# intel/neural-compressor

Hardware: AMD Instinct MI355X
Metric: llama2_7b_gptq_int4_g128_quantize_wall_clock (lower is better)
Workload: dtype bf16

## Files before the change

### include/inc_mi355x.h

```cpp
#ifndef INC_MI355X_H_
#define INC_MI355X_H_

#include <stdint.h>

#ifdef __cplusplus
extern "C" {
#endif

#define INC_OK 0
#define INC_ERR_BAD_ARG (-1)
#define INC_ERR_UNSUPPORTED (-2)
#define INC_ERR_LAUNCH (-3)
#define INC_ERR_WORKSPACE (-4)

#define INC_F32 0
#define INC_F16 1
#define INC_BF16 2

#define INC_SCHEME_ASYM 0
#define INC_SCHEME_SYM 1

typedef void* inc_stream_t;

int inc_abi_version(void);
// ... 122 lines not shown
int inc_gptq_hessian_accum_routed(const void* a, int xdtype, int mode, const int32_t* route, int64_t T, int top_k, int64_t E,
                                  int64_t K, float* H, int64_t* rows, inc_stream_t stream);

int inc_gptq_hessian_finalize(float* H, int64_t K, float percdamp, uint8_t* dead, void* workspace,
                              inc_stream_t stream);

int inc_gptq_prepare_weight(const void* w, int wdtype, float* out, const uint8_t* dead, int64_t N,
                            int64_t K, inc_stream_t stream);

int inc_gptq_find_params(const float* w, int64_t N, int64_t K, int64_t col0, int group_size,
                         int ngroups, int bits, int sym, float* scale, float* zero, int64_t G,
                         int64_t g0, inc_stream_t stream);

int inc_gptq_find_params_mse(const float* w, int64_t N, int64_t K, int64_t col0, int group_size,
                             int ngroups, int bits, int sym, int grid, float maxshrink, float norm,
                             float* scale, float* zero, int64_t G, int64_t g0, inc_stream_t stream);

int inc_gptq_quant_block(const float* w, const float* Hinv, const float* scale, const float* zero,
                         uint8_t* codes, void* q_out, int q_dtype, float* err, int64_t N, int64_t K,
                         int64_t G, int64_t i1, int count, int group_size, int bits,
                         inc_stream_t stream);

int inc_gptq_quant_block_params(const float* w, const float* Hinv, float* scale, float* zero,
                                uint8_t* codes, void* q_out, int q_dtype, float* err, int64_t N, int64_t K,
                                int64_t G, int64_t i1, int count, int group_size, int bits, int sym,
                                inc_stream_t stream);

int inc_gptq_lazy_update(float* w, const float* Hinv, const float* err, int64_t N, int64_t K,
                         int64_t i1, int count, inc_stream_t stream);

int inc_gptq_lazy_update_cols(float* w, const float* Hinv, const float* err, int64_t N, int64_t K,
                              int64_t i1, int count, int64_t col_begin, int64_t col_end,
                              inc_stream_t stream);

#define INC_GPTQ_DYNAMIC_GROUPS 1
#define INC_GPTQ_MSE 2
#define INC_GPTQ_NO_LOOKAHEAD 4
#define INC_GPTQ_NO_FUSED_PARAMS 8
int inc_gptq_quantize_layer(float* w, const float* Hinv, float* scale, float* zero, int64_t G,
                            const float* loop_scale, const float* loop_zero, int64_t loop_G, uint8_t* codes,
                            void* q_out, int q_dtype, float* err_ws, int64_t N, int64_t K, int group_size,
                            int kernel_group_size, int block_size, int bits, int sym, int flags,
                            inc_stream_t stream, inc_stream_t aux_stream);

int inc_chol_diag_block(float* A, int64_t lda, int n, float* Linv, int64_t ldi, int32_t* info, int tag,
                        inc_stream_t stream);

int64_t inc_gptq_inverse_factor_workspace_bytes(int64_t K, int flags);
int inc_gptq_inverse_factor(const float* H, int64_t K, float* U, void* workspace, int64_t workspace_bytes, int32_t* info,
                            int flags, inc_stream_t stream, inc_stream_t aux_stream);

int inc_awq_act_abs_sum(const void* x, int xdtype, int64_t T, int64_t K, float* out,
                        inc_stream_t stream);
int64_t inc_awq_weight_scale_workspace_bytes(int64_t N, int64_t K, int group_size);
int inc_awq_weight_scale(const void* w, int wdtype, int64_t N, int64_t K, int group_size, float* out,
                         void* workspace, int64_t workspace_bytes, inc_stream_t stream);

int inc_awq_repack(const int32_t* awq_qweight, const int32_t* awq_qzeros, int64_t K, int64_t N, int64_t G, int bits,
                   int32_t* qweight, int32_t* qzeros, inc_stream_t stream);

int64_t inc_w8a8_gemm_workspace_bytes(int64_t M, int64_t N, int64_t K);
int inc_sq_channel_minmax(const void* x, int xdtype, int64_t T, int64_t K, int64_t ld, float* mn, float* mx,
                          inc_stream_t stream);
int inc_sq_weight_col_absmax(const void* w, int wdtype, int64_t N, int64_t K, float* out, inc_stream_t stream);
int inc_sq_cal_scale(const float* amax_x, const float* amax_w, int64_t K, float alpha, float weight_max_lb, float* scale,
                     inc_stream_t stream);
int inc_sq_quant_weight(const void* w, int wdtype, int64_t N, int64_t K, int64_t Kp, const float* smooth, int8_t* qw,
                        float* w_scale, int32_t* rowsum, inc_stream_t stream);
int inc_sq_quant_act(const void* x, int xdtype, int64_t M, int64_t K, int64_t Kp, const float* in_scale, float sx, float zp,
                     int8_t* out, inc_stream_t stream);
int inc_w8a8_gemm(const int8_t* xq, const int8_t* wq, const float* alpha, const int32_t* corr, const void* bias, void* y,
                  int ydtype, int64_t M, int64_t N, int64_t K, void* workspace, int64_t workspace_bytes,
                  inc_stream_t stream);

int inc_probe_hbm_triad(float* a, const float* b, const float* c, float s, int64_t n, inc_stream_t stream);
int inc_probe_hbm_copy(void* dst, const void* src, int64_t bytes, int variant, inc_stream_t stream);
int inc_probe_mfma_bf16(const void* src, float* sink, int blocks, int iters, double* flops_out, inc_stream_t stream);
int inc_trace_marker(int id, inc_stream_t stream);

int inc_fwd_silu_mul(const void* gate, const void* up, void* out, int64_t n, int dtype, inc_stream_t stream);
int inc_fwd_rope(const void* q, const void* k, const void* cos, const void* sin, void* q_out, void* k_out, int64_t B, int64_t Hq,
                 int64_t Hk, int64_t T, int64_t D, const int64_t* strides, int64_t cs_batch, int dtype, inc_stream_t stream);
int inc_fwd_rmsnorm(const void* x, const void* w, void* out, int64_t rows, int64_t cols, float eps, int dtype, inc_stream_t stream);

#ifdef __cplusplus
}
#endif
#endif
```

### neural_compressor_amd/_lib.py

```python

import ctypes
import os
from ctypes import c_char_p, c_float, c_int, c_int64, c_void_p

_HERE = os.path.dirname(os.path.abspath(__file__))
LIB_PATH = os.path.join(_HERE, "libinc_mi355x.so")
ABI_VERSION = 12

INC_OK = 0
INC_F32, INC_F16, INC_BF16 = 0, 1, 2
INC_SCHEME_ASYM, INC_SCHEME_SYM = 0, 1

_P = c_void_p
SIGNATURES = {
    "inc_abi_version": (c_int, []),
    "inc_error_string": (c_char_p, [c_int]),
    "inc_target_arch": (c_char_p, []),
    "inc_pack_rows": (c_int, [_P, _P, c_int64, c_int64, c_int, c_int, _P]),
    "inc_unpack_rows": (c_int, [_P, _P, c_int64, c_int64, c_int, c_int, c_int, _P]),
    "inc_woq_pack": (c_int, [_P, c_int, _P, _P, _P, _P, _P, c_int64, c_int64, c_int64, c_int, c_int, _P]),
    "inc_woq_unpack": (c_int, [_P, _P, _P, _P, c_int64, c_int64, c_int64, c_int, _P, _P, _P]),
    "inc_woq_dequant": (c_int, [_P, _P, _P, _P, _P, c_int, c_int64, c_int64, c_int64, c_int, c_int, _P]),
    "inc_dequant_ints": (c_int, [_P, _P, c_int, _P, _P, _P, c_int, c_int64, c_int64, c_int64, c_int, _P]),
    "inc_woq_gemm_workspace_bytes": (c_int64, [c_int64, c_int64, c_int64]),
    "inc_woq_gemm": (
        c_int,
        [_P, c_int, _P, _P, _P, _P, _P, _P, c_int64, c_int64, c_int64, c_int64, c_int, c_int, _P, c_int64, _P],
    ),
    "inc_woq_gemm_route": (
        c_int,
        [c_int64, c_int64, c_int64, c_int, c_int, c_int, c_int, _P, _P, _P, _P, c_int64, _P, _P, _P, _P, _P, _P],
    ),
    "inc_woq_gemm_perm": (
        c_int,
        [_P, c_int, _P, _P, _P, _P, _P, _P, c_int64, c_int64, c_int64, c_int64, c_int, c_int, _P, c_int64, _P],
    ),
    "inc_woq_gemm_lut_workspace_bytes": (c_int64, [c_int64, c_int64, c_int64]),
    "inc_woq_gemm_lut": (
        c_int,
        [_P, c_int, _P, c_int64, _P, _P, c_int, c_int, _P, c_int64, _P, _P, c_int64, c_int64, c_int64, c_int64, c_int, _P, c_int64, _P],
    ),
    "inc_moe_route_bytes": (c_int64, [c_int64, c_int, c_int64]),
    "inc_moe_route": (c_int, [_P, c_int, c_int64, c_int, c_int64, _P, c_int64, _P]),
    "inc_woq_moe_gemm_workspace_bytes": (c_int64, [c_int, c_int64, c_int, c_int64, c_int64, c_int64]),
    "inc_woq_moe_gemm": (
        c_int,
        [c_int, _P, c_int, _P, _P, _P, _P, _P, c_int, _P, c_int64, c_int, c_int64, c_int64, c_int64, c_int64, c_int, _P, c_int64, _P],
    ),
    "inc_moe_combine": (c_int, [_P, _P, _P, c_int, c_int64, c_int, c_int64, c_int64, _P]),
    "inc_woq_gemm_multi_workspace_bytes": (c_int64, [c_int, c_int64, _P, c_int64]),
    "inc_woq_gemm_multi": (c_int, [c_int, _P, c_int, _P, _P, _P, _P, _P, c_int64, _P, c_int64, c_int, c_int, _P, c_int64, _P]),
    "inc_woq_gemm_multi_perm": (c_int, [c_int, _P, c_int, _P, _P, _P, _P, _P, _P, c_int64, _P, c_int64, c_int, c_int, _P, c_int64, _P]),
    "inc_woq_gemm_gated_workspace_bytes": (c_int64, [c_int64, c_int64, c_int64]),
    "inc_woq_gemm_gated": (
        c_int,
        [_P, c_int, _P, _P, _P, _P, _P, _P, _P, _P, _P, c_int64, c_int64, c_int64, c_int, c_int, c_int, _P, c_int64, _P],
    ),
    "inc_woq_gemv_anyw_slices": (c_int, [c_int64, c_int64, c_int64, c_int]),
    "inc_woq_gemv_anyw_workspace_bytes": (c_int64, [c_int64, c_int64, c_int64, c_int]),
    "inc_woq_gemv_anyw": (c_int, [_P, c_int, _P, _P, _P, _P, _P, c_int64, c_int64, c_int64, c_int64, c_int, c_int, _P, c_int64, _P]),
    "inc_woq_gemv_anyw_perm": (c_int, [_P, c_int, _P, _P, _P, _P, _P, _P, c_int64, c_int64, c_int64, c_int64, c_int, c_int, _P, c_int64, _P]),
    "inc_woq_gemv_anyw_multi_workspace_bytes": (c_int64, [c_int, c_int64, _P, c_int64, c_int]),
    "inc_woq_gemv_anyw_multi": (c_int, [c_int, _P, c_int, _P, _P, _P, _P, _P, _P, c_int64, _P, c_int64, c_int, c_int, _P, c_int64, _P]),
    "inc_groupwise_quant": (
        c_int,
        [_P, c_int, _P, _P, _P, _P, c_int64, c_int64, c_int, c_int, c_int, c_float, c_int, _P],
    ),
    "inc_codebook_quant": (c_int, [_P, c_int, _P, _P, _P, c_int64, c_int64, c_int, _P, _P, c_int, c_float, _P]),
    "inc_codebook_quant_with_scale": (c_int, [_P, c_int, _P, _P, _P, c_int64, c_int64, c_int, _P, _P, c_int, c_float, _P, _P]),
    "inc_mse_accumulate_workspace_bytes": (c_int64, []),
    "inc_mse_accumulate": (c_int, [_P, _P, c_int, c_int64, _P, _P, _P]),
    "inc_gptq_hessian_accum": (c_int, [_P, c_int, c_int64, c_int64, c_int64, _P, c_float, c_float, _P]),
    "inc_gptq_hessian_accum_multi": (c_int, [c_int, _P, c_int, c_int64, _P, _P, _P, _P, _P, _P, c_int64, _P]),
    "inc_gptq_hessian_accum_multi_workspace_bytes": (c_int64, []),
    "inc_gptq_hessian_accum_routed": (c_int, [_P, c_int, c_int, _P, c_int64, c_int, c_int64, c_int64, _P, _P, _P]),
    "inc_gptq_hessian_finalize": (c_int, [_P, c_int64, c_float, _P, _P, _P]),
    "inc_gptq_prepare_weight": (c_int, [_P, c_int, _P, _P, c_int64, c_int64, _P]),
    "inc_gptq_find_params": (
        c_int,
        [_P, c_int64, c_int64, c_int64, c_int, c_int, c_int, c_int, _P, _P, c_int64, c_int64, _P],
    ),
    "inc_sq_channel_minmax": (c_int, [_P, c_int, c_int64, c_int64, c_int64, _P, _P, _P]),
    "inc_sq_weight_col_absmax": (c_int, [_P, c_int, c_int64, c_int64, _P, _P]),
    "inc_sq_cal_scale": (c_int, [_P, _P, c_int64, c_float, c_float, _P, _P]),
    "inc_sq_quant_weight": (c_int, [_P, c_int, c_int64, c_int64, c_int64, _P, _P, _P, _P, _P]),
    "inc_sq_quant_act": (c_int, [_P, c_int, c_int64, c_int64, c_int64, _P, c_float, c_float, _P, _P]),
    "inc_w8a8_gemm_workspace_bytes": (c_int64, [c_int64, c_int64, c_int64]),
    "inc_w8a8_gemm": (c_int, [_P, _P, _P, _P, _P, _P, c_int, c_int64, c_int64, c_int64, _P, c_int64, _P]),
    "inc_awq_repack": (c_int, [_P, _P, c_int64, c_int64, c_int64, c_int, _P, _P, _P]),
    "inc_gptq_find_params_mse": (
        c_int,
        [_P, c_int64, c_int64, c_int64, c_int, c_int, c_int, c_int, c_int, c_float, c_float, _P, _P, c_int64, c_int64, _P],
    ),
    "inc_gptq_quant_block": (
        c_int,
        [_P, _P, _P, _P, _P, _P, c_int, _P, c_int64, c_int64, c_int64, c_int64, c_int, c_int, c_int, _P],
    ),
    "inc_gptq_quant_block_params": (c_int, [_P, _P, _P, _P, _P, _P, c_int, _P, c_int64, c_int64, c_int64, c_int64, c_int, c_int, c_int, c_int, _P]),
    "inc_gptq_lazy_update": (c_int, [_P, _P, _P, c_int64, c_int64, c_int64, c_int, _P]),
    "inc_gptq_lazy_update_cols": (c_int, [_P, _P, _P, c_int64, c_int64, c_int64, c_int, c_int64, c_int64, _P]),
    "inc_probe_hbm_triad": (c_int, [_P, _P, _P, c_float, c_int64, _P]),
    "inc_probe_hbm_copy": (c_int, [_P, _P, c_int64, c_int, _P]),
    "inc_probe_mfma_bf16": (c_int, [_P, _P, c_int, c_int, _P, _P]),
    "inc_trace_marker": (c_int, [c_int, _P]),
    "inc_gptq_quantize_layer": (c_int, [_P, _P, _P, _P, c_int64, _P, _P, c_int64, _P, _P, c_int, _P, c_int64, c_int64, c_int, c_int, c_int,
                                        c_int, c_int, c_int, _P, _P]),
    "inc_chol_diag_block": (c_int, [_P, c_int64, c_int, _P, c_int64, _P, c_int, _P]),
    "inc_gptq_inverse_factor_workspace_bytes": (c_int64, [c_int64, c_int]),
    "inc_gptq_inverse_factor": (c_int, [_P, c_int64, _P, _P, c_int64, _P, c_int, _P, _P]),
    "inc_awq_act_abs_sum": (c_int, [_P, c_int, c_int64, c_int64, _P, _P]),
    "inc_awq_weight_scale_workspace_bytes": (c_int64, [c_int64, c_int64, c_int]),
    "inc_awq_weight_scale": (c_int, [_P, c_int, c_int64, c_int64, c_int, _P, _P, c_int64, _P]),
    "inc_fwd_silu_mul": (c_int, [_P, _P, _P, c_int64, c_int, _P]),
    "inc_fwd_rope": (c_int, [_P, _P, _P, _P, _P, _P, c_int64, c_int64, c_int64, c_int64, c_int64, _P, c_int64, c_int, _P]),
    "inc_fwd_rmsnorm": (c_int, [_P, _P, _P, c_int64, c_int64, c_float, c_int, _P]),
}


class IncLibraryError(RuntimeError):
    """Raised when libinc_mi355x.so is missing, stale, or a call returns an INC_ERR_* code."""


def _load():
    if not os.path.exists(LIB_PATH):
        raise IncLibraryError(
            f"{LIB_PATH} not found. The MI355X HIP extension is mandatory (there is no CPU fallback): "
            "build it with `python -c 'import __graft_entry__ as g; g.build()'` or "
            "`make -C neural_compressor_amd/csrc`."
        )
    lib = ctypes.CDLL(LIB_PATH)
    for name, (restype, argtypes) in SIGNATURES.items():
        try:
            fn = getattr(lib, name)
        except AttributeError as e:
            raise IncLibraryError(f"{LIB_PATH} does not export `{name}`; rebuild the extension") from e
        fn.restype = restype
        fn.argtypes = argtypes
    got = lib.inc_abi_version()
    if got != ABI_VERSION:
        raise IncLibraryError(f"ABI mismatch: library reports {got}, bindings expect {ABI_VERSION}; rebuild")
    return lib


lib = _load()


def check(code, what):
    if code != INC_OK:
        msg = lib.inc_error_string(code).decode()
        raise IncLibraryError(f"{what} failed: {msg} (code {code})")
```

### neural_compressor_amd/csrc/fwd_elementwise.hip

```cpp
#include "common.hpp"

namespace {

typedef uint32_t u32x4 __attribute__((ext_vector_type(4)));

template <int DT>
__device__ __forceinline__ uint16_t t_round(float f) {
  if constexpr (DT == INC_BF16) {
    uint32_t u = __float_as_uint(f);
    if ((u & 0x7fffffffu) > 0x7f800000u) return 0x7FC0;
    u += 0x7fffu + ((u >> 16) & 1u);
    return static_cast<uint16_t>(u >> 16);
  } else {
    return f32_to_f16_bits(f);
  }
}
template <int DT>
__device__ __forceinline__ float t_f32(uint16_t b) {
  if constexpr (DT == INC_BF16) return bf16_bits_to_f32(b);
  else return f16_bits_to_f32(b);
}
template <int DT>
__device__ __forceinline__ float t_rf(float f) { return t_f32<DT>(t_round<DT>(f)); }

template <int DT>
__device__ __forceinline__ void unpack8(const u32x4 v, float (&e)[8]) {
#pragma unroll
  for (int i = 0; i < 4; ++i) {
    e[2 * i] = t_f32<DT>(static_cast<uint16_t>(v[i] & 0xffffu));
    e[2 * i + 1] = t_f32<DT>(static_cast<uint16_t>(v[i] >> 16));
  }
}
__device__ __forceinline__ u32x4 pack8(const uint16_t (&b)[8]) {
  u32x4 v;
#pragma unroll
  for (int i = 0; i < 4; ++i) v[i] = static_cast<uint32_t>(b[2 * i]) | (static_cast<uint32_t>(b[2 * i + 1]) << 16);
  return v;
}
__device__ __forceinline__ u32x4 ld_nt(const void* p, int64_t i16) { return __builtin_nontemporal_load(static_cast<const u32x4*>(p) + i16); }
__device__ __forceinline__ void st_nt(void* p, int64_t i16, u32x4 v) { __builtin_nontemporal_store(v, static_cast<u32x4*>(p) + i16); }

template <int DT>
__device__ __forceinline__ uint16_t silu_mul_one(float g, float u) {
#pragma clang fp contract(off)
  const float s = t_rf<DT>(g / (1.0f + expf(-g)));
  return t_round<DT>(s * u);
}

template <int DT>
__global__ __launch_bounds__(256) void fwd_silu_mul_kernel(const void* __restrict__ gate, const void* __restrict__ up, void* __restrict__ out, int64_t n) {
  const int64_t n8 = n >> 3;
  const int64_t i = (int64_t)blockIdx.x * 256 + threadIdx.x;
  if (i < n8) {
    float g[8], u[8];
    unpack8<DT>(ld_nt(gate, i), g);
    unpack8<DT>(ld_nt(up, i), u);
    uint16_t r[8];
#pragma unroll
    for (int e = 0; e < 8; ++e) r[e] = silu_mul_one<DT>(g[e], u[e]);
    st_nt(out, i, pack8(r));
  } else {
    const int64_t e = n8 * 8 + (i - n8);
    if (e < n) {
      const uint16_t* g = static_cast<const uint16_t*>(gate);
      const uint16_t* u = static_cast<const uint16_t*>(up);
      static_cast<uint16_t*>(out)[e] = silu_mul_one<DT>(t_f32<DT>(g[e]), t_f32<DT>(u[e]));
    }
  }
}

struct RopeStrides {
  int64_t q[3], k[3], qo[3], ko[3];
};

template <int DT>
__global__ __launch_bounds__(256) void fwd_rope_kernel(const void* __restrict__ q, const void* __restrict__ k, const void* __restrict__ cosp,
                                                       const void* __restrict__ sinp, void* __restrict__ q_out, void* __restrict__ k_out,
                                                       uint32_t total, uint32_t Hq, uint32_t Hk, uint32_t T, uint32_t D, uint32_t cs_batch,
                                                       RopeStrides st) {
#pragma clang fp contract(off)
  const uint32_t idx = blockIdx.x * 256u + threadIdx.x;
  if (idx >= total) return;
  const uint32_t d16 = D >> 4, H = Hq + Hk;
  const uint32_t dc = idx % d16;
  uint32_t r = idx / d16;
  const uint32_t hh = r % H;
  r /= H;
  const uint32_t t = r % T, b = r / T;
  const bool is_k = hh >= Hq;
  const uint32_t h = is_k ? hh - Hq : hh;
  const int64_t* si = is_k ? st.k : st.q;
  const int64_t* so = is_k ? st.ko : st.qo;
  const char* src = static_cast<const char*>(is_k ? k : q);
  char* dst = static_cast<char*>(is_k ? k_out : q_out);
  const int64_t in_off = (int64_t)b * si[0] + (int64_t)h * si[1] + (int64_t)t * si[2] + dc * 8;
  const int64_t out_off = (int64_t)b * so[0] + (int64_t)h * so[1] + (int64_t)t * so[2] + dc * 8;
  const int64_t cs_off = ((int64_t)(cs_batch == 1 ? 0 : b) * T + t) * D + dc * 8;
  const int64_t half = D >> 1;

  float lo[8], hi[8], c_lo[8], c_hi[8], s_lo[8], s_hi[8];
  unpack8<DT>(ld_nt(src, in_off >> 3), lo);
  unpack8<DT>(ld_nt(src, (in_off + half) >> 3), hi);
  unpack8<DT>(static_cast<const u32x4*>(cosp)[cs_off >> 3], c_lo);
  unpack8<DT>(static_cast<const u32x4*>(cosp)[(cs_off + half) >> 3], c_hi);
  unpack8<DT>(static_cast<const u32x4*>(sinp)[cs_off >> 3], s_lo);
  unpack8<DT>(static_cast<const u32x4*>(sinp)[(cs_off + half) >> 3], s_hi);
  uint16_t o_lo[8], o_hi[8];
#pragma unroll
  for (int e = 0; e < 8; ++e) {
    o_lo[e] = t_round<DT>(t_rf<DT>(lo[e] * c_lo[e]) + t_rf<DT>(-hi[e] * s_lo[e]));
    o_hi[e] = t_round<DT>(t_rf<DT>(hi[e] * c_hi[e]) + t_rf<DT>(lo[e] * s_hi[e]));
  }
  st_nt(dst, out_off >> 3, pack8(o_lo));
  st_nt(dst, (out_off + half) >> 3, pack8(o_hi));
}

template <int DT, int WAVES, int J>
__global__ __launch_bounds__(WAVES == 1 ? 256 : 512) void fwd_rmsnorm_kernel(const void* __restrict__ x, const void* __restrict__ w, void* __restrict__ out,
                                                                              int64_t rows, int cols, float eps, float factor) {
#pragma clang fp contract(off)
  constexpr int HALVES = (WAVES == 1 ? 256 : 512) / 32, ROWS_PER_BLOCK = HALVES / WAVES;
  __shared__ float part[ROWS_PER_BLOCK][8];
  const int p = threadIdx.x & 31, hw = threadIdx.x >> 5;
  const int rb = hw / WAVES, tw = hw % WAVES;
  const int64_t row = (int64_t)blockIdx.x * ROWS_PER_BLOCK + rb;
  const bool live = row < rows;
  const int pieces = cols >> 3;
  const int64_t base = (live ? row : 0) * (int64_t)pieces;
  const int first = p + 32 * tw;

  u32x4 v[J];
#pragma unroll
  for (int j = 0; j < J; ++j) {
    const int u = first + 32 * WAVES * j;
    if (live && u < pieces) v[j] = ld_nt(x, base + u);
  }
  float a[4] = {0.f, 0.f, 0.f, 0.f}, b[4] = {0.f, 0.f, 0.f, 0.f};
#pragma unroll
  for (int j = 0; j < J; ++j) {
    const int u = first + 32 * WAVES * j;
    if (live && u < pieces) {
      float e[8];
      unpack8<DT>(v[j], e);
#pragma unroll
      for (int i = 0; i < 4; ++i) {
        a[i] = a[i] + e[i] * e[i];
        b[i] = b[i] + e[4 + i] * e[4 + i];
      }
    }
  }
  float s = (((a[0] + a[1]) + a[2]) + a[3]) + (((b[0] + b[1]) + b[2]) + b[3]);
#pragma unroll
  for (int o = 1; o < 32; o <<= 1) s = s + __shfl_down(s, o, 32);
  if constexpr (WAVES == 1) {
    s = __shfl(s, 0, 32);
  } else {
    if (p == 0) part[rb][tw] = s;
    __syncthreads();
    const float* q = part[rb];
    s = ((q[0] + q[4]) + (q[2] + q[6])) + ((q[1] + q[5]) + (q[3] + q[7]));
  }
  if (!live) return;
  const float mean = s * factor;
  const float rs = static_cast<float>(::rsqrt(static_cast<double>(mean + eps)));
#pragma unroll
  for (int j = 0; j < J; ++j) {
    const int u = first + 32 * WAVES * j;
    if (u < pieces) {
      float e[8], g[8];
      unpack8<DT>(v[j], e);
      unpack8<DT>(static_cast<const u32x4*>(w)[u], g);
      uint16_t r[8];
#pragma unroll
      for (int i = 0; i < 8; ++i) r[i] = t_round<DT>(g[i] * t_rf<DT>(e[i] * rs));
      st_nt(out, base + u, pack8(r));
    }
  }
}

template <int DT, int WAVES, int J>
void rmsnorm_launch(const void* x, const void* w, void* out, int64_t rows, int cols, float eps, float factor, hipStream_t s) {
  constexpr int THREADS = WAVES == 1 ? 256 : 512, ROWS_PER_BLOCK = THREADS / 32 / WAVES;
  fwd_rmsnorm_kernel<DT, WAVES, J><<<(unsigned)ceil_div64(rows, ROWS_PER_BLOCK), THREADS, 0, s>>>(x, w, out, rows, cols, eps, factor);
}

inline bool aligned16(const void* p) { return (reinterpret_cast<uintptr_t>(p) & 15u) == 0; }

}

extern "C" {

int inc_fwd_silu_mul(const void* gate, const void* up, void* out, int64_t n, int dtype, inc_stream_t stream) {
  INC_CHECK_ARG(gate && up && out && n > 0);
  if (dtype != INC_BF16 && dtype != INC_F16) return INC_ERR_UNSUPPORTED;
  if (!aligned16(gate) || !aligned16(up) || !aligned16(out)) return INC_ERR_UNSUPPORTED;
  const int64_t blocks = ceil_div64((n >> 3) + (n & 7), 256);
  if (blocks > 0x7fffffff) return INC_ERR_UNSUPPORTED;
  if (dtype == INC_BF16) fwd_silu_mul_kernel<INC_BF16><<<(unsigned)blocks, 256, 0, inc_s(stream)>>>(gate, up, out, n);
  else fwd_silu_mul_kernel<INC_F16><<<(unsigned)blocks, 256, 0, inc_s(stream)>>>(gate, up, out, n);
  INC_LAUNCH_RETURN();
}

int inc_fwd_rope(const void* q, const void* k, const void* cos, const void* sin, void* q_out, void* k_out, int64_t B, int64_t Hq,
                 int64_t Hk, int64_t T, int64_t D, const int64_t* strides, int64_t cs_batch, int dtype, inc_stream_t stream) {
  INC_CHECK_ARG(q && k && cos && sin && q_out && k_out && strides && B > 0 && Hq > 0 && Hk > 0 && T > 0 && D > 0);
  INC_CHECK_ARG(cs_batch == 1 || cs_batch == B);
  if (dtype != INC_BF16 && dtype != INC_F16) return INC_ERR_UNSUPPORTED;
  if (D % 16 != 0) return INC_ERR_UNSUPPORTED;
  RopeStrides st;
  for (int i = 0; i < 3; ++i) {
    st.q[i] = strides[i];
    st.k[i] = strides[3 + i];
    st.qo[i] = strides[6 + i];
    st.ko[i] = strides[9 + i];
  }
  for (int i = 0; i < 12; ++i)
    if (strides[i] < 0 || strides[i] % 8 != 0) return INC_ERR_UNSUPPORTED;
  if (!aligned16(q) || !aligned16(k) || !aligned16(cos) || !aligned16(sin) || !aligned16(q_out) || !aligned16(k_out)) return INC_ERR_UNSUPPORTED;
  if (B >= (1ll << 31) || T >= (1ll << 31) || Hq + Hk >= (1ll << 31)) return INC_ERR_UNSUPPORTED;
  const double items = (double)B * (double)T * (double)(Hq + Hk) * (double)(D / 16);
  if (items >= 2147483648.0 - 256.0) return INC_ERR_UNSUPPORTED;
  const uint32_t total = (uint32_t)(B * T * (Hq + Hk) * (D / 16));
  const unsigned blocks = (total + 255u) / 256u;
  if (dtype == INC_BF16)
    fwd_rope_kernel<INC_BF16><<<blocks, 256, 0, inc_s(stream)>>>(q, k, cos, sin, q_out, k_out, total, (uint32_t)Hq, (uint32_t)Hk, (uint32_t)T, (uint32_t)D, (uint32_t)cs_batch, st);
  else
    fwd_rope_kernel<INC_F16><<<blocks, 256, 0, inc_s(stream)>>>(q, k, cos, sin, q_out, k_out, total, (uint32_t)Hq, (uint32_t)Hk, (uint32_t)T, (uint32_t)D, (uint32_t)cs_batch, st);
  INC_LAUNCH_RETURN();
}

int inc_fwd_rmsnorm(const void* x, const void* w, void* out, int64_t rows, int64_t cols, float eps, int dtype, inc_stream_t stream) {
  INC_CHECK_ARG(x && w && out && rows > 0 && cols > 0);
  if (dtype != INC_BF16 && dtype != INC_F16) return INC_ERR_UNSUPPORTED;
  if (rows < 8 || cols % 8 != 0 || cols < 256 || cols > 16384 || rows >= (1ll << 40)) return INC_ERR_UNSUPPORTED;
  if (!aligned16(x) || !aligned16(w) || !aligned16(out)) return INC_ERR_UNSUPPORTED;
  if (ceil_div64(rows, 2) > 0x7fffffff) return INC_ERR_UNSUPPORTED;
  const float factor = static_cast<float>(rows) / static_cast<float>(rows * cols);
  const int c = (int)cols;
  hipStream_t s = inc_s(stream);
#define INC_RMS(W, JJ)                                                                        \
  do {                                                                                        \
    if (dtype == INC_BF16) rmsnorm_launch<INC_BF16, W, JJ>(x, w, out, rows, c, eps, factor, s); \
    else rmsnorm_launch<INC_F16, W, JJ>(x, w, out, rows, c, eps, factor, s);                    \
  } while (0)
  if (cols <= 8128) {
    if (cols <= 2048) INC_RMS(1, 8);
    else if (cols <= 4096) INC_RMS(1, 16);
    else if (cols <= 6144) INC_RMS(1, 24);
    else INC_RMS(1, 32);
  } else {
    INC_RMS(8, 8);
  }
#undef INC_RMS
  INC_LAUNCH_RETURN();
}

}
```

### neural_compressor_amd/ops.py

```python

import torch

from ._lib import INC_BF16, INC_F16, INC_F32, INC_SCHEME_ASYM, INC_SCHEME_SYM, check, lib

_DT = {torch.float32: INC_F32, torch.float16: INC_F16, torch.bfloat16: INC_BF16}


def dtype_code(dtype):
    try:
        return _DT[dtype]
    except KeyError as e:
        raise TypeError(f"unsupported floating dtype {dtype}; expected fp32/fp16/bf16") from e


def _dev(*tensors):
    dev = None
    for t in tensors:
        if t is None:
            continue
        if t.device.type != "cuda":
            raise RuntimeError(
                f"MI355X op got a tensor on {t.device}; tensors must be resident in HBM (device 'cuda' = HIP). "
                "There is no CPU fallback."
            )
# ... 1061 lines not shown
    check(rc, "inc_gptq_lazy_update_cols")
    return True


def probe_hbm_triad(a, b, c, s):
    dev = _dev(a, b, c)
    with torch.cuda.device(dev):
        check(lib.inc_probe_hbm_triad(_ptr(a), _ptr(b), _ptr(c), float(s), a.numel(), _stream()), "inc_probe_hbm_triad")


def probe_hbm_copy(dst, src, variant=0):
    dev = _dev(dst, src)
    nbytes = src.numel() * src.element_size()
    assert nbytes == dst.numel() * dst.element_size() and nbytes % 16 == 0
    with torch.cuda.device(dev):
        check(lib.inc_probe_hbm_copy(_ptr(dst), _ptr(src), nbytes, int(variant), _stream()), "inc_probe_hbm_copy")
    return dst


def probe_mfma_bf16(src, sink, blocks, iters):
    import ctypes

    dev = _dev(src, sink)
    assert src.numel() * src.element_size() >= 65536 and sink.numel() >= blocks * 256
    flops = ctypes.c_double(0.0)
    with torch.cuda.device(dev):
        check(lib.inc_probe_mfma_bf16(_ptr(src), _ptr(sink), int(blocks), int(iters), ctypes.byref(flops), _stream()), "inc_probe_mfma_bf16")
    return flops.value


def _fwd_call(fn, name, args):
    rc = fn(*args)
    if rc == -2:
        return False
    check(rc, name)
    return True


def fwd_silu_mul(gate, up):
    dev = _dev(gate, up)
    if gate.shape != up.shape or gate.dtype != up.dtype or gate.numel() == 0:
        return None
    out = torch.empty_like(gate)
    with torch.cuda.device(dev):
        ok = _fwd_call(lib.inc_fwd_silu_mul, "inc_fwd_silu_mul", (_ptr(gate), _ptr(up), _ptr(out), gate.numel(), dtype_code(gate.dtype), _stream()))
    return out if ok else None


def fwd_rmsnorm(x, weight, eps):
    dev = _dev(x, weight)
    cols = x.shape[-1]
    if x.dtype != weight.dtype or weight.shape != (cols,) or x.numel() == 0:
        return None
    out = torch.empty_like(x)
    with torch.cuda.device(dev):
        ok = _fwd_call(lib.inc_fwd_rmsnorm, "inc_fwd_rmsnorm",
                       (_ptr(x), _ptr(weight), _ptr(out), x.numel() // cols, cols, float(eps), dtype_code(x.dtype), _stream()))
    return out if ok else None


def fwd_rope(q, k, cos, sin, q_out_strides, k_out_strides):
    import ctypes

    for t in (q, k, cos, sin):
        if t.device.type != "cuda" or t.device != q.device or t.dtype != q.dtype:
            return None
    if q.dim() != 4 or k.dim() != 4 or cos.dim() != 3 or cos.shape != sin.shape or not cos.is_contiguous() or not sin.is_contiguous():
        return None
    B, Hq, T, D = q.shape
    if k.shape[0] != B or k.shape[2] != T or k.shape[3] != D or cos.shape[1:] != (T, D) or cos.shape[0] not in (1, B):
        return None
    if q.numel() == 0 or k.numel() == 0 or q.stride(3) != 1 or k.stride(3) != 1 or q_out_strides[3] != 1 or k_out_strides[3] != 1:
        return None
    q_out = torch.empty_strided(q.shape, q_out_strides, dtype=q.dtype, device=q.device)
    k_out = torch.empty_strided(k.shape, k_out_strides, dtype=k.dtype, device=k.device)
    strides = (ctypes.c_int64 * 12)(*q.stride()[:3], *k.stride()[:3], *q_out_strides[:3], *k_out_strides[:3])
    with torch.cuda.device(q.device):
        ok = _fwd_call(lib.inc_fwd_rope, "inc_fwd_rope",
                       (_ptr(q), _ptr(k), _ptr(cos), _ptr(sin), _ptr(q_out), _ptr(k_out), B, Hq, k.shape[1], T, D, strides, cos.shape[0],
                        dtype_code(q.dtype), _stream()))
    return (q_out, k_out) if ok else None


_HIP_RT = None


def cu_masked_stream(device, mask_words):
    global _HIP_RT
    import ctypes

    try:
        if _HIP_RT is None:
            _HIP_RT = ctypes.CDLL("libamdhip64.so")
        st = ctypes.c_void_p()
        arr = (ctypes.c_uint32 * len(mask_words))(*mask_words)
        with torch.cuda.device(device):
            if _HIP_RT.hipExtStreamCreateWithCUMask(ctypes.byref(st), len(mask_words), arr) != 0 or not st.value:
                return None
            return torch.cuda.ExternalStream(st.value, device=device)
    except Exception:
        return None


def trace_marker(marker_id, device=None):
    with torch.cuda.device(device if device is not None else torch.cuda.current_device()):
        check(lib.inc_trace_marker(int(marker_id), _stream()), "inc_trace_marker")


GPTQ_DYNAMIC_GROUPS, GPTQ_MSE, GPTQ_NO_LOOKAHEAD, GPTQ_NO_FUSED_PARAMS = 1, 2, 4, 8


def gptq_quantize_layer(w32, hinv, scale, zero, loop_scale, loop_zero, codes, q_out, err_ws, group_size, kernel_group_size, block_size,
                        bits, sym, flags, aux_stream=None):
    dev = _dev(w32, hinv, scale, zero, codes, q_out, err_ws)
    N, K = w32.shape
    assert err_ws.dtype == torch.float32 and err_ws.numel() >= 2 * N * 128
    with torch.cuda.device(dev):
        check(
            lib.inc_gptq_quantize_layer(
                _ptr(w32), _ptr(hinv), _ptr(scale), _ptr(zero), scale.shape[1], _ptr(loop_scale), _ptr(loop_zero),
                loop_scale.shape[1] if loop_scale is not None else scale.shape[1], _ptr(codes), _ptr(q_out),
                dtype_code(q_out.dtype) if q_out is not None else INC_F32, _ptr(err_ws), N, K, int(group_size), int(kernel_group_size),
                int(block_size), int(bits), 1 if sym else 0, int(flags), _stream(),
                aux_stream.cuda_stream if aux_stream is not None else None,
            ),
            "inc_gptq_quantize_layer",
        )


def chol_diag_block(A_view, Linv_view, info, tag):
    dev = A_view.device
    if dev.type != "cuda" or Linv_view.device != dev:
        raise RuntimeError("chol_diag_block needs HBM-resident views")
    n = A_view.shape[0]
    assert A_view.shape == (n, n) and Linv_view.shape == (n, n) and A_view.stride(1) == 1 and Linv_view.stride(1) == 1
    assert A_view.dtype == torch.float32 and Linv_view.dtype == torch.float32
    with torch.cuda.device(dev):
        check(
            lib.inc_chol_diag_block(A_view.data_ptr(), A_view.stride(0), n, Linv_view.data_ptr(), Linv_view.stride(0),
                                    _ptr(info), int(tag), _stream()),
            "inc_chol_diag_block",
        )


def gptq_inverse_factor(H, aux_stream=None, flags=0):
    dev = _dev(H)
    K = H.shape[0]
    assert H.shape == (K, K) and H.dtype == torch.float32 and H.is_contiguous()
    U = torch.empty((K, K), dtype=torch.float32, device=dev)
    info = torch.empty(1, dtype=torch.int32, device=dev)
    wsb = int(lib.inc_gptq_inverse_factor_workspace_bytes(K, int(flags)))
    ws = torch.empty(wsb, dtype=torch.uint8, device=dev)
    aux = aux_stream.cuda_stream if aux_stream is not None else None
    with torch.cuda.device(dev):
        check(lib.inc_gptq_inverse_factor(_ptr(H), K, _ptr(U), _ptr(ws), wsb, _ptr(info), int(flags), _stream(), aux), "inc_gptq_inverse_factor")
    return U, info


def awq_act_abs_sum(x2d, out):
    dev = _dev(x2d, out)
    T, K = x2d.shape
    with torch.cuda.device(dev):
        check(lib.inc_awq_act_abs_sum(_ptr(x2d), dtype_code(x2d.dtype), T, K, _ptr(out), _stream()), "inc_awq_act_abs_sum")
    return out


# ... 111 lines not shown
```

### neural_compressor_amd/torch/algorithms/weight_only/fused_forward.py

```python

import contextlib
import os
import threading

import torch

from .... import ops
from ....common.utils import logger

ENV_SWITCH = "INC_MI355X_GPTQ_FUSED_FORWARD"
_DTYPES = (torch.bfloat16, torch.float16)

try:
    from transformers.models.llama import modeling_llama as _llama

    _ORIG_ROPE = _llama.apply_rotary_pos_emb
    if getattr(_ORIG_ROPE, "__module__", None) != _llama.__name__ or getattr(_ORIG_ROPE, "__name__", None) != "apply_rotary_pos_emb":
        _ORIG_ROPE = None
except Exception:
    _llama, _ORIG_ROPE = None, None


def switch_on():
    return os.environ.get(ENV_SWITCH, "1") != "0"


def _usable(*tensors):
    t0 = tensors[0]
    for t in tensors:
        if not isinstance(t, torch.Tensor) or t.device.type != "cuda" or t.device != t0.device or t.dtype != t0.dtype:
            return False
        if t.requires_grad and torch.is_grad_enabled():
            return False
    return t0.dtype in _DTYPES


def _same_bits(a, b):
    if a.shape != b.shape or a.dtype != b.dtype or a.stride() != b.stride():
        return False
    return bool(torch.equal(a.view(torch.int16), b.view(torch.int16)))


def silu_mul(gate, up):
    if not (_usable(gate, up) and gate.is_contiguous() and up.is_contiguous()):
        return None
    return ops.fwd_silu_mul(gate, up)


def rmsnorm(x, weight, eps):
    if not (_usable(x, weight) and x.dim() >= 2 and x.is_contiguous() and weight.is_contiguous()):
        return None
    return ops.fwd_rmsnorm(x, weight, eps)


def rmsnorm_routed(module, x):
    out = rmsnorm(x, module.weight, module.variance_epsilon)
    if out is not None:
        return out, "fused"
    return type(module).forward(module, x), "eager"


_ROPE_STRIDES = {}


def _eager_rope_strides(q, k, cos, sin):
    key = (q.shape, q.stride(), k.shape, k.stride(), cos.shape, cos.stride(), sin.stride(), q.dtype)
    got = _ROPE_STRIDES.get(key)
    if got is None:
        mq, mk, mc, ms = (torch.empty_strided(t.shape, t.stride(), dtype=t.dtype, device="meta") for t in (q, k, cos, sin))
        eq, ek = _ORIG_ROPE(mq, mk, mc, ms)
        got = (tuple(eq.stride()), tuple(ek.stride())) if eq.shape == q.shape and ek.shape == k.shape else False
        if len(_ROPE_STRIDES) > 256:
            _ROPE_STRIDES.clear()
        _ROPE_STRIDES[key] = got
    return got


def rope(q, k, cos, sin):
    if _ORIG_ROPE is None or not _usable(q, k, cos, sin) or q.dim() != 4 or k.dim() != 4 or cos.dim() != 3 or sin.dim() != 3:
        return None
    if q.stride(3) != 1 or k.stride(3) != 1 or not cos.is_contiguous() or not sin.is_contiguous():
        return None
    strides = _eager_rope_strides(q, k, cos, sin)
    if not strides:
        return None
    return ops.fwd_rope(q, k, cos, sin, strides[0], strides[1])


_tls = threading.local()
_rope_lock = threading.Lock()
_rope_users = 0


def _rope_entry(q, k, cos, sin, *args, **kwargs):
    active = getattr(_tls, "active", None)
    unsqueeze_dim = args[0] if args else kwargs.get("unsqueeze_dim", 1)
    if active is None or len(args) > 1 or (kwargs and set(kwargs) != {"unsqueeze_dim"}) or unsqueeze_dim != 1:
        return _ORIG_ROPE(q, k, cos, sin, *args, **kwargs)
    state, block = active

    def check(fused, ref):
        return _same_bits(fused[0], ref[0]) and _same_bits(fused[1], ref[1])

    shape = (tuple(q.shape), tuple(k.shape), tuple(cos.shape)) if isinstance(q, torch.Tensor) and isinstance(k, torch.Tensor) and isinstance(cos, torch.Tensor) else None
    return state.dispatch("rotary embedding", block, getattr(q, "dtype", None), shape, lambda: rope(q, k, cos, sin),
                          lambda: _ORIG_ROPE(q, k, cos, sin, *args, **kwargs), check)


def _is_silu(act):
    if type(act) is torch.nn.SiLU:
        return not act.inplace
    try:
        from transformers.activations import SiLUActivation
    except Exception:
        return False
    return type(act) is SiLUActivation


class FusedForward:

    def __init__(self):
        self.disabled = False
        self.verified = set()
        self.fused_calls = 0

    def dispatch(self, op, block, dtype, shape, fused_fn, eager_fn, same=_same_bits):
        if self.disabled or shape is None:
            return eager_fn()
        key = (op, type(block), dtype, shape)
        fused = fused_fn()
        if fused is None:
            return eager_fn()
        self.fused_calls += 1
        if key in self.verified:
            return fused
        ref = eager_fn()
        if same(fused, ref):
            self.verified.add(key)
        else:
            self.disabled = True
            logger.warning(f"GPTQ fused forward: the fused {op} kernel does not reproduce eager bit for bit on this model's tensors "
                           f"({dtype}, shape {shape}); the fused forward is off for the rest of the run")
        return ref

    def _norm_forward(self, block, m):
        def forward(hidden_states):
            eager = lambda: type(m).forward(m, hidden_states)
            if not isinstance(hidden_states, torch.Tensor):
                return eager()
            return self.dispatch("RMSNorm", block, hidden_states.dtype, tuple(hidden_states.shape),
                                 lambda: rmsnorm(hidden_states, m.weight, m.variance_epsilon), eager)

        return forward

# ... 50 lines not shown
```

Measured before the change: 7.742.

## Reuse cos/sin across heads in fused RoPE and vectorize bf16 rounding

The RoPE kernel now gives each thread a (token, 16-head group, d-chunk) slice. It loads cos/sin once and loops over heads with a prefetch of the next head's data, where before every head re-read cos/sin. The bf16 pack/unpack paths use vector bf16 conversion with a wave-wide NaN fallback, and plain shifts instead of per-element conversion calls. A probe kernel checks rounding equivalence, and the stride detection for contiguous RoPE outputs is adjusted. These elementwise ops are a small part of the GPTQ calibration forward, so the overall effect is likely limited, and rounding mismatches would disable the fused path.

```diff
diff --git a/include/inc_mi355x.h b/include/inc_mi355x.h
--- a/include/inc_mi355x.h
+++ b/include/inc_mi355x.h
@@ -228,6 +228,7 @@
 int inc_fwd_rope(const void* q, const void* k, const void* cos, const void* sin, void* q_out, void* k_out, int64_t B, int64_t Hq,
                  int64_t Hk, int64_t T, int64_t D, const int64_t* strides, int64_t cs_batch, int dtype, inc_stream_t stream);
 int inc_fwd_rmsnorm(const void* x, const void* w, void* out, int64_t rows, int64_t cols, float eps, int dtype, inc_stream_t stream);
+int inc_probe_round_bf16(uint16_t* out, uint32_t first_bits, int64_t n, inc_stream_t stream);
 
 #ifdef __cplusplus
 }
diff --git a/neural_compressor_amd/_lib.py b/neural_compressor_amd/_lib.py
--- a/neural_compressor_amd/_lib.py
+++ b/neural_compressor_amd/_lib.py
@@ -1,7 +1,7 @@
 
 import ctypes
 import os
-from ctypes import c_char_p, c_float, c_int, c_int64, c_void_p
+from ctypes import c_char_p, c_float, c_int, c_int64, c_uint32, c_void_p
 
 _HERE = os.path.dirname(os.path.abspath(__file__))
 LIB_PATH = os.path.join(_HERE, "libinc_mi355x.so")
@@ -114,6 +114,7 @@
     "inc_fwd_silu_mul": (c_int, [_P, _P, _P, c_int64, c_int, _P]),
     "inc_fwd_rope": (c_int, [_P, _P, _P, _P, _P, _P, c_int64, c_int64, c_int64, c_int64, c_int64, _P, c_int64, c_int, _P]),
     "inc_fwd_rmsnorm": (c_int, [_P, _P, _P, c_int64, c_int64, c_float, c_int, _P]),
+    "inc_probe_round_bf16": (c_int, [_P, c_uint32, c_int64, _P]),
 }
 
 
diff --git a/neural_compressor_amd/csrc/fwd_elementwise.hip b/neural_compressor_amd/csrc/fwd_elementwise.hip
--- a/neural_compressor_amd/csrc/fwd_elementwise.hip
+++ b/neural_compressor_amd/csrc/fwd_elementwise.hip
@@ -3,6 +3,8 @@
 namespace {
 
 typedef uint32_t u32x4 __attribute__((ext_vector_type(4)));
+typedef float f32x2 __attribute__((ext_vector_type(2)));
+typedef __bf16 bf16x2 __attribute__((ext_vector_type(2)));
 
 template <int DT>
 __device__ __forceinline__ uint16_t t_round(float f) {
@@ -27,15 +29,43 @@
 __device__ __forceinline__ void unpack8(const u32x4 v, float (&e)[8]) {
 #pragma unroll
   for (int i = 0; i < 4; ++i) {
-    e[2 * i] = t_f32<DT>(static_cast<uint16_t>(v[i] & 0xffffu));
-    e[2 * i + 1] = t_f32<DT>(static_cast<uint16_t>(v[i] >> 16));
-  }
-}
-__device__ __forceinline__ u32x4 pack8(const uint16_t (&b)[8]) {
+    if constexpr (DT == INC_BF16) {
+      e[2 * i] = __uint_as_float(v[i] << 16);
+      e[2 * i + 1] = __uint_as_float(v[i] & 0xffff0000u);
+    } else {
+      e[2 * i] = t_f32<DT>(static_cast<uint16_t>(v[i] & 0xffffu));
+      e[2 * i + 1] = t_f32<DT>(static_cast<uint16_t>(v[i] >> 16));
+    }
+  }
+}
+
+template <int DT>
+__device__ __forceinline__ u32x4 round8(const float (&f)[8]) {
   u32x4 v;
-#pragma unroll
-  for (int i = 0; i < 4; ++i) v[i] = static_cast<uint32_t>(b[2 * i]) | (static_cast<uint32_t>(b[2 * i + 1]) << 16);
+  if constexpr (DT == INC_BF16) {
+    bool nan = false;
+#pragma unroll
+    for (int i = 0; i < 4; ++i) {
+      const f32x2 p = {f[2 * i], f[2 * i + 1]};
+      const bf16x2 h = __builtin_convertvector(p, bf16x2);
+      uint32_t w;
+      __builtin_memcpy(&w, &h, 4);
+      v[i] = w;
+      nan |= __builtin_isunordered(f[2 * i], f[2 * i + 1]);
+    }
+    if (__builtin_amdgcn_ballot_w64(nan) != 0) {
+#pragma unroll
+      for (int i = 0; i < 4; ++i) v[i] = static_cast<uint32_t>(t_round<DT>(f[2 * i])) | (static_cast<uint32_t>(t_round<DT>(f[2 * i + 1])) << 16);
+    }
+  } else {
+#pragma unroll
+    for (int i = 0; i < 4; ++i) v[i] = static_cast<uint32_t>(t_round<DT>(f[2 * i])) | (static_cast<uint32_t>(t_round<DT>(f[2 * i + 1])) << 16);
+  }
   return v;
+}
+template <int DT>
+__device__ __forceinline__ void rf8(float (&f)[8]) {
+  unpack8<DT>(round8<DT>(f), f);
 }
 __device__ __forceinline__ u32x4 ld_nt(const void* p, int64_t i16) { return __builtin_nontemporal_load(static_cast<const u32x4*>(p) + i16); }
 __device__ __forceinline__ void st_nt(void* p, int64_t i16, u32x4 v) { __builtin_nontemporal_store(v, static_cast<u32x4*>(p) + i16); }
@@ -52,13 +82,16 @@
   const int64_t n8 = n >> 3;
   const int64_t i = (int64_t)blockIdx.x * 256 + threadIdx.x;
   if (i < n8) {
+#pragma clang fp contract(off)
     float g[8], u[8];
     unpack8<DT>(ld_nt(gate, i), g);
     unpack8<DT>(ld_nt(up, i), u);
-    uint16_t r[8];
-#pragma unroll
-    for (int e = 0; e < 8; ++e) r[e] = silu_mul_one<DT>(g[e], u[e]);
-    st_nt(out, i, pack8(r));
+#pragma unroll
+    for (int e = 0; e < 8; ++e) g[e] = g[e] / (1.0f + expf(-g[e]));
+    rf8<DT>(g);
+#pragma unroll
+    for (int e = 0; e < 8; ++e) g[e] = g[e] * u[e];
+    st_nt(out, i, round8<DT>(g));
   } else {
     const int64_t e = n8 * 8 + (i - n8);
     if (e < n) {
@@ -72,47 +105,73 @@
 struct RopeStrides {
   int64_t q[3], k[3], qo[3], ko[3];
 };
+constexpr int ROPE_HEADS = 16;
+
+template <int DT>
+__device__ __forceinline__ void rope_heads(const void* __restrict__ src, void* __restrict__ dst, int64_t in_off, int64_t out_off, int64_t in_step,
+                                           int64_t out_step, int h0, int h1, int64_t half, const float (&c_lo)[8], const float (&c_hi)[8],
+                                           const float (&s_lo)[8], const float (&s_hi)[8]) {
+#pragma clang fp contract(off)
+  if (h0 >= h1) return;
+  u32x4 n_lo = ld_nt(src, in_off >> 3), n_hi = ld_nt(src, (in_off + half) >> 3);
+  for (int h = h0; h < h1; ++h, out_off += out_step) {
+    float lo[8], hi[8], a[8], r[8];
+    unpack8<DT>(n_lo, lo);
+    unpack8<DT>(n_hi, hi);
+    in_off += in_step;
+    if (h + 1 < h1) {
+      n_lo = ld_nt(src, in_off >> 3);
+      n_hi = ld_nt(src, (in_off + half) >> 3);
+    }
+#pragma unroll
+    for (int e = 0; e < 8; ++e) {
+      a[e] = lo[e] * c_lo[e];
+      r[e] = -hi[e] * s_lo[e];
+    }
+    rf8<DT>(a);
+    rf8<DT>(r);
+#pragma unroll
+    for (int e = 0; e < 8; ++e) a[e] = a[e] + r[e];
+    st_nt(dst, out_off >> 3, round8<DT>(a));
+#pragma unroll
+    for (int e = 0; e < 8; ++e) {
+      a[e] = hi[e] * c_hi[e];
+      r[e] = lo[e] * s_hi[e];
+    }
+    rf8<DT>(a);
+    rf8<DT>(r);
+#pragma unroll
+    for (int e = 0; e < 8; ++e) a[e] = a[e] + r[e];
+    st_nt(dst, (out_off + half) >> 3, round8<DT>(a));
+  }
+}
 
 template <int DT>
 __global__ __launch_bounds__(256) void fwd_rope_kernel(const void* __restrict__ q, const void* __restrict__ k, const void* __restrict__ cosp,
                                                        const void* __restrict__ sinp, void* __restrict__ q_out, void* __restrict__ k_out,
-                                                       uint32_t total, uint32_t Hq, uint32_t Hk, uint32_t T, uint32_t D, uint32_t cs_batch,
-                                                       RopeStrides st) {
-#pragma clang fp contract(off)
-  const uint32_t idx = blockIdx.x * 256u + threadIdx.x;
-  if (idx >= total) return;
-  const uint32_t d16 = D >> 4, H = Hq + Hk;
-  const uint32_t dc = idx % d16;
-  uint32_t r = idx / d16;
-  const uint32_t hh = r % H;
-  r /= H;
-  const uint32_t t = r % T, b = r / T;
-  const bool is_k = hh >= Hq;
-  const uint32_t h = is_k ? hh - Hq : hh;
-  const int64_t* si = is_k ? st.k : st.q;
-  const int64_t* so = is_k ? st.ko : st.qo;
-  const char* src = static_cast<const char*>(is_k ? k : q);
-  char* dst = static_cast<char*>(is_k ? k_out : q_out);
-  const int64_t in_off = (int64_t)b * si[0] + (int64_t)h * si[1] + (int64_t)t * si[2] + dc * 8;
-  const int64_t out_off = (int64_t)b * so[0] + (int64_t)h * so[1] + (int64_t)t * so[2] + dc * 8;
-  const int64_t cs_off = ((int64_t)(cs_batch == 1 ? 0 : b) * T + t) * D + dc * 8;
+                                                       int B, int Hq, int Hk, int T, int D, int cs_batch, RopeStrides st) {
+  const int t = (int)(blockIdx.x * blockDim.y + threadIdx.y);
+  if (t >= T) return;
+  const int d16 = D >> 4;
   const int64_t half = D >> 1;
-
-  float lo[8], hi[8], c_lo[8], c_hi[8], s_lo[8], s_hi[8];
-  unpack8<DT>(ld_nt(src, in_off >> 3), lo);
-  unpack8<DT>(ld_nt(src, (in_off + half) >> 3), hi);
-  unpack8<DT>(static_cast<const u32x4*>(cosp)[cs_off >> 3], c_lo);
-  unpack8<DT>(static_cast<const u32x4*>(cosp)[(cs_off + half) >> 3], c_hi);
-  unpack8<DT>(static_cast<const u32x4*>(sinp)[cs_off >> 3], s_lo);
-  unpack8<DT>(static_cast<const u32x4*>(sinp)[(cs_off + half) >> 3], s_hi);
-  uint16_t o_lo[8], o_hi[8];
-#pragma unroll
-  for (int e = 0; e < 8; ++e) {
-    o_lo[e] = t_round<DT>(t_rf<DT>(lo[e] * c_lo[e]) + t_rf<DT>(-hi[e] * s_lo[e]));
-    o_hi[e] = t_round<DT>(t_rf<DT>(hi[e] * c_hi[e]) + t_rf<DT>(lo[e] * s_hi[e]));
-  }
-  st_nt(dst, out_off >> 3, pack8(o_lo));
-  st_nt(dst, (out_off + half) >> 3, pack8(o_hi));
+  const int g0 = (int)blockIdx.z * ROPE_HEADS, g1 = min(g0 + ROPE_HEADS, Hq + Hk);
+  const int q0 = min(g0, Hq), q1 = min(g1, Hq), k0 = max(g0, Hq) - Hq, k1 = max(g1, Hq) - Hq;
+  for (int b = (int)blockIdx.y; b < B; b += (int)gridDim.y) {
+    for (int dc = (int)threadIdx.x; dc < d16; dc += (int)blockDim.x) {
+      const int64_t cs_off = ((int64_t)(cs_batch == 1 ? 0 : b) * T + t) * D + dc * 8;
+      float c_lo[8], c_hi[8], s_lo[8], s_hi[8];
+      unpack8<DT>(static_cast<const u32x4*>(cosp)[cs_off >> 3], c_lo);
+      unpack8<DT>(static_cast<const u32x4*>(cosp)[(cs_off + half) >> 3], c_hi);
+      unpack8<DT>(static_cast<const u32x4*>(sinp)[cs_off >> 3], s_lo);
+      unpack8<DT>(static_cast<const u32x4*>(sinp)[(cs_off + half) >> 3], s_hi);
+      rope_heads<DT>(q, q_out, (int64_t)b * st.q[0] + (int64_t)q0 * st.q[1] + (int64_t)t * st.q[2] + dc * 8,
+                     (int64_t)b * st.qo[0] + (int64_t)q0 * st.qo[1] + (int64_t)t * st.qo[2] + dc * 8, st.q[1], st.qo[1], q0, q1, half, c_lo, c_hi,
+                     s_lo, s_hi);
+      rope_heads<DT>(k, k_out, (int64_t)b * st.k[0] + (int64_t)k0 * st.k[1] + (int64_t)t * st.k[2] + dc * 8,
+                     (int64_t)b * st.ko[0] + (int64_t)k0 * st.ko[1] + (int64_t)t * st.ko[2] + dc * 8, st.k[1], st.ko[1], k0, k1, half, c_lo, c_hi,
+                     s_lo, s_hi);
+    }
+  }
 }
 
 template <int DT, int WAVES, int J>
@@ -170,10 +229,12 @@
       float e[8], g[8];
       unpack8<DT>(v[j], e);
       unpack8<DT>(static_cast<const u32x4*>(w)[u], g);
-      uint16_t r[8];
-#pragma unroll
-      for (int i = 0; i < 8; ++i) r[i] = t_round<DT>(g[i] * t_rf<DT>(e[i] * rs));
-      st_nt(out, base + u, pack8(r));
+#pragma unroll
+      for (int i = 0; i < 8; ++i) e[i] = e[i] * rs;
+      rf8<DT>(e);
+#pragma unroll
+      for (int i = 0; i < 8; ++i) e[i] = g[i] * e[i];
+      st_nt(out, base + u, round8<DT>(e));
     }
   }
 }
@@ -182,6 +243,20 @@
 void rmsnorm_launch(const void* x, const void* w, void* out, int64_t rows, int cols, float eps, float factor, hipStream_t s) {
   constexpr int THREADS = WAVES == 1 ? 256 : 512, ROWS_PER_BLOCK = THREADS / 32 / WAVES;
   fwd_rmsnorm_kernel<DT, WAVES, J><<<(unsigned)ceil_div64(rows, ROWS_PER_BLOCK), THREADS, 0, s>>>(x, w, out, rows, cols, eps, factor);
+}
+
+__global__ __launch_bounds__(256) void probe_round_bf16_kernel(uint16_t* __restrict__ out, uint32_t first_bits, int64_t n8) {
+  const int64_t i = (int64_t)blockIdx.x * 256 + threadIdx.x;
+  if (i >= n8) return;
+  float f[8];
+#pragma unroll
+  for (int e = 0; e < 8; ++e) f[e] = __uint_as_float(first_bits + (uint32_t)(i * 8 + e));
+  reinterpret_cast<u32x4*>(out)[i] = round8<INC_BF16>(f);
+  rf8<INC_BF16>(f);
+  u32x4 v;
+#pragma unroll
+  for (int e = 0; e < 4; ++e) v[e] = (__float_as_uint(f[2 * e]) >> 16) | (__float_as_uint(f[2 * e + 1]) & 0xffff0000u);
+  reinterpret_cast<u32x4*>(out)[n8 + i] = v;
 }
 
 inline bool aligned16(const void* p) { return (reinterpret_cast<uintptr_t>(p) & 15u) == 0; }
@@ -217,15 +292,17 @@
   for (int i = 0; i < 12; ++i)
     if (strides[i] < 0 || strides[i] % 8 != 0) return INC_ERR_UNSUPPORTED;
   if (!aligned16(q) || !aligned16(k) || !aligned16(cos) || !aligned16(sin) || !aligned16(q_out) || !aligned16(k_out)) return INC_ERR_UNSUPPORTED;
-  if (B >= (1ll << 31) || T >= (1ll << 31) || Hq + Hk >= (1ll << 31)) return INC_ERR_UNSUPPORTED;
-  const double items = (double)B * (double)T * (double)(Hq + Hk) * (double)(D / 16);
-  if (items >= 2147483648.0 - 256.0) return INC_ERR_UNSUPPORTED;
-  const uint32_t total = (uint32_t)(B * T * (Hq + Hk) * (D / 16));
-  const unsigned blocks = (total + 255u) / 256u;
+  if (B >= (1ll << 31) || T >= (1ll << 31) || Hq + Hk >= (1ll << 31) || D >= (1ll << 31)) return INC_ERR_UNSUPPORTED;
+  int lanes = 1;
+  while (lanes < 8 && lanes < D / 16) lanes *= 2;
+  const dim3 block(lanes, 256 / lanes);
+  const int64_t runs = ceil_div64(Hq + Hk, ROPE_HEADS);
+  if (runs > 65535) return INC_ERR_UNSUPPORTED;
+  const dim3 grid((unsigned)ceil_div64(T, block.y), (unsigned)(B < 65535 ? B : 65535), (unsigned)runs);
   if (dtype == INC_BF16)
-    fwd_rope_kernel<INC_BF16><<<blocks, 256, 0, inc_s(stream)>>>(q, k, cos, sin, q_out, k_out, total, (uint32_t)Hq, (uint32_t)Hk, (uint32_t)T, (uint32_t)D, (uint32_t)cs_batch, st);
+    fwd_rope_kernel<INC_BF16><<<grid, block, 0, inc_s(stream)>>>(q, k, cos, sin, q_out, k_out, (int)B, (int)Hq, (int)Hk, (int)T, (int)D, (int)cs_batch, st);
   else
-    fwd_rope_kernel<INC_F16><<<blocks, 256, 0, inc_s(stream)>>>(q, k, cos, sin, q_out, k_out, total, (uint32_t)Hq, (uint32_t)Hk, (uint32_t)T, (uint32_t)D, (uint32_t)cs_batch, st);
+    fwd_rope_kernel<INC_F16><<<grid, block, 0, inc_s(stream)>>>(q, k, cos, sin, q_out, k_out, (int)B, (int)Hq, (int)Hk, (int)T, (int)D, (int)cs_batch, st);
   INC_LAUNCH_RETURN();
 }
 
@@ -255,4 +332,11 @@
   INC_LAUNCH_RETURN();
 }
 
-}
+int inc_probe_round_bf16(uint16_t* out, uint32_t first_bits, int64_t n, inc_stream_t stream) {
+  INC_CHECK_ARG(out && n > 0);
+  if (n % 8 != 0 || (int64_t)first_bits + n > (1ll << 32) || !aligned16(out)) return INC_ERR_UNSUPPORTED;
+  probe_round_bf16_kernel<<<(unsigned)ceil_div64(n >> 3, 256), 256, 0, inc_s(stream)>>>(out, first_bits, n >> 3);
+  INC_LAUNCH_RETURN();
+}
+
+}
diff --git a/neural_compressor_amd/ops.py b/neural_compressor_amd/ops.py
--- a/neural_compressor_amd/ops.py
+++ b/neural_compressor_amd/ops.py
@@ -1167,6 +1167,14 @@
     return (q_out, k_out) if ok else None
 
 
+def probe_round_bf16(out, first_bits):
+    dev = _dev(out)
+    assert out.dtype == torch.int16 and out.dim() == 2 and out.shape[0] == 2 and out.is_contiguous()
+    with torch.cuda.device(dev):
+        check(lib.inc_probe_round_bf16(_ptr(out), int(first_bits), out.shape[1], _stream()), "inc_probe_round_bf16")
+    return out
+
+
 _HIP_RT = None
 
 
diff --git a/neural_compressor_amd/torch/algorithms/weight_only/fused_forward.py b/neural_compressor_amd/torch/algorithms/weight_only/fused_forward.py
--- a/neural_compressor_amd/torch/algorithms/weight_only/fused_forward.py
+++ b/neural_compressor_amd/torch/algorithms/weight_only/fused_forward.py
@@ -69,7 +69,10 @@
     if got is None:
         mq, mk, mc, ms = (torch.empty_strided(t.shape, t.stride(), dtype=t.dtype, device="meta") for t in (q, k, cos, sin))
         eq, ek = _ORIG_ROPE(mq, mk, mc, ms)
-        got = (tuple(eq.stride()), tuple(ek.stride())) if eq.shape == q.shape and ek.shape == k.shape else False
+        def strides(t):
+            return tuple(torch.empty(t.shape, device="meta").stride()) if t.is_contiguous() else tuple(t.stride())
+
+        got = (strides(eq), strides(ek)) if eq.shape == q.shape and ek.shape == k.shape else False
         if len(_ROPE_STRIDES) > 256:
             _ROPE_STRIDES.clear()
         _ROPE_STRIDES[key] = got
```

Result: faster. 7.665 (median of 6 runs) (-1.0%).
